# microsoft/VidTok

Measured on NVIDIA H100. Metric: frames/sec encode+decode, kl_causal_488 17x256x256, higher is better.
Workload: dtype bf16

## Files before the change

### vidtok_b200/csrc/conv_tc.cu

```cuda
#include <cuda.h>

#include <cstdio>
#include <cstdlib>
#include <cstring>
#include <mutex>
#include <string>
#include <type_traits>

#include "common.cuh"
#include "kernels.h"
#include "tc_host.h"
#include "tc_ptx.cuh"

namespace vt {

namespace {

thread_local std::string g_tc_err;

struct TcParams {
  int B, To, Ho, Wo, Co, Ti;
  int BW, BH, BT;
  int tilesW, tilesH, tilesT;
  int num_n_tiles, BN;
  long long num_tiles;
  int kt, kh, kw, Ci, num_kc;
  int st, pt, ph, pw, to_off;
  int sp;
  int t_mode, cacheT;
  int stages;
  const float* bias;
  int res_mode;
  const bf16* res;
  long long rsB, rsT, rsH, rsW;
  int resT, res_t_mode, res_pool_off;
  const bf16* res_cache;
  float ra, rb;
  void* out;
  long long osB, osT, osH, osW, osC;
  int out_f32;
  int Co_real;
  int w_batched;
  int ln_mode, ln_silu;
  const float* ln_gamma;
  const float* ln_beta;
  void* out2;
  int res_mma;
  int halo, hP, a_stages;
  uint32_t halo_bytes;
  int split, a_lo, b_lo, o_lo;
  float acc_scale;
  int kparts;
  int reg_mode, reg_zc, reg_sample;
  const float* reg_noise;
  float* reg_z;
  int* reg_idx;
  double* reg_kl;
  FsqConst reg_fsq;
  uint32_t misc_off;
  int stage_out;
  uint32_t stage_smem;
  uint32_t stage_off;
  int half_dim, half_ext;
  int relu;
};

struct TcMaps {
  CUtensorMap a[4];
  CUtensorMap c;
  CUtensorMap b;
  CUtensorMap r;
  CUtensorMap e;
  CUtensorMap o, o2;
};

constexpr int kConsumerWarps = 8;
constexpr int kProducerWarp = kConsumerWarps;
constexpr int kThreads = (kConsumerWarps + 4) * 32;
constexpr int kABytes = 128 * 128;
constexpr uint32_t kBarTurn = 3, kBarBias = 5, kBarStage = 7;
constexpr uint32_t kStageOutBytes = 64 * 128;

__host__ __device__ constexpr bool ping_pong(int BN, bool split) { return !split && (BN == 64 || BN == 128); }

using namespace tcx;

struct TileCoord {
  int b, t0, h0, w0, n0;
};
__device__ __forceinline__ TileCoord decode_tile(const TcParams& p, long long tile) {
  TileCoord c;
  const int nt = (int)(tile % p.num_n_tiles);
  long long m = tile / p.num_n_tiles;
  const int tw = (int)(m % p.tilesW); m /= p.tilesW;
  const int th = (int)(m % p.tilesH); m /= p.tilesH;
  const int tt = (int)(m % p.tilesT);
  c.b = (int)(m / p.tilesT);
  c.t0 = tt * p.BT; c.h0 = th * p.BH; c.w0 = tw * p.BW; c.n0 = nt * p.BN;
  return c;
}
__device__ __forceinline__ bool tap_time(const TcParams& p, const TileCoord& tc, int a, int& tv, bool& from_cache) {
  tv = (tc.t0 + p.to_off) * p.st + a - p.pt;
  from_cache = false;
  if (tv + p.BT <= 0) {
    if (p.t_mode == 0) return false;
    if (p.t_mode == 1) { tv = 0; return true; }
    from_cache = true;
    tv = p.cacheT + tv;
    return true;
  }
  return true;
}
__device__ __forceinline__ int tile_taps(const TcParams& p, const TileCoord& tc) {
  int n = 0;
  for (int a = 0; a < p.kt; ++a) {
    int tv;
    bool from_cache;
    if (tap_time(p, tc, a, tv, from_cache)) ++n;
  }
  return n;
}

__device__ __forceinline__ float quad_sum(float v) {
  v += __shfl_xor_sync(0xffffffffu, v, 1);
  v += __shfl_xor_sync(0xffffffffu, v, 2);
  return v;
}

template <int BN, bool kSplit, bool kStage = false>
__global__ void __launch_bounds__(kThreads, 1)
conv_tc_kernel(const __grid_constant__ TcMaps maps, const TcParams p) {
  extern __shared__ uint8_t smem_raw[];
  const uint32_t smem_base = (smem_u32(smem_raw) + 1023u) & ~1023u;
  uint8_t* smem_gen = smem_raw + (smem_base - smem_u32(smem_raw));
  const int warp = threadIdx.x >> 5, lane = threadIdx.x & 31;
  const uint32_t a_bytes = kABytes;
  constexpr uint32_t b_bytes = (uint32_t)BN * 128u;
  constexpr uint32_t kPl = kSplit ? 2u : 1u;
  const uint32_t stage_bytes = kPl * (p.halo ? b_bytes : a_bytes + b_bytes);
  const uint32_t win_bytes = kPl * p.halo_bytes;
  const uint32_t ring_base = smem_base + (p.halo ? (uint32_t)p.a_stages * win_bytes : 0u);
  const uint32_t bar_base = ring_base + p.stages * stage_bytes + p.stage_smem;
  auto full_bar = [&](int s) { return bar_base + 8u * s; };
  auto empty_bar = [&](int s) { return bar_base + 8u * (p.stages + s); };
  auto fullA_bar = [&](int s) { return bar_base + 8u * (2 * p.stages + s); };
  auto emptyA_bar = [&](int s) { return bar_base + 8u * (2 * p.stages + p.a_stages + s); };
  constexpr bool kPingPong = ping_pong(BN, kSplit);
  float* sbias = reinterpret_cast<float*>(smem_gen + p.misc_off);
  float* rowbuf = sbias + 2 * 768;

  if (threadIdx.x == 0) {
    constexpr uint32_t readers = kPingPong ? kConsumerWarps / 2 : kConsumerWarps;
    for (int s = 0; s < p.stages; ++s) {
      mbar_init(full_bar(s), 1);
      mbar_init(empty_bar(s), readers);
    }
    for (int s = 0; s < p.a_stages; ++s) {
      mbar_init(fullA_bar(s), 1);
      mbar_init(emptyA_bar(s), readers);
    }
    asm volatile("fence.mbarrier_init.release.cluster;" ::: "memory");
  }
  __syncthreads();

  const int nsp = p.kh * p.kw;
  const int num_kc = p.num_kc, nstages = p.stages;
  const bool halo = p.halo != 0;
  const int res_steps = p.res_mma ? BN / 64 : 0;

  if (warp >= kProducerWarp) {
    asm volatile("setmaxnreg.dec.sync.aligned.u32 40;" ::: "memory");
    if (warp != kProducerWarp) return;
    const bool el = elect_one();
    if (el) {
      prefetch_tmap(&maps.a[0]);
      prefetch_tmap(&maps.b);
      if (p.sp == 2) { prefetch_tmap(&maps.a[1]); prefetch_tmap(&maps.a[2]); prefetch_tmap(&maps.a[3]); }
      if (p.t_mode == 2) prefetch_tmap(&maps.c);
      if (p.res_mma) { prefetch_tmap(&maps.r); prefetch_tmap(&maps.e); }
    }
    int stage = 0, sA = 0;
    uint32_t phase = 0, phA = 0;
    auto acquire = [&](uint32_t bytes) {
      mbar_wait(empty_bar(stage), phase ^ 1u);
      if (el) mbar_expect_tx(full_bar(stage), bytes);
    };
    auto advance = [&]() { if (++stage == nstages) { stage = 0; phase ^= 1u; } };
    auto load_b_planes = [&](uint32_t dst, const CUtensorMap* m, int kcol, int n, int wb_) {
      tma_load_3d(dst, m, full_bar(stage), kcol, n, wb_);
      if constexpr (kSplit) tma_load_3d(dst + b_bytes, m, full_bar(stage), p.b_lo + kcol, n, wb_);
    };
    auto load_window = [&](const CUtensorMap* m, int c0, int lo_off, int cw, int ch, int ct, int cb) {
      mbar_wait(emptyA_bar(sA), phA ^ 1u);
      if (el) {
        mbar_expect_tx(fullA_bar(sA), win_bytes);
        tma_load_5d(smem_base + (uint32_t)sA * win_bytes, m, fullA_bar(sA), c0, cw, ch, ct, cb);
        if constexpr (kSplit) tma_load_5d(smem_base + (uint32_t)sA * win_bytes + p.halo_bytes, m, fullA_bar(sA), lo_off + c0, cw, ch, ct, cb);
      }
      if (++sA == p.a_stages) { sA = 0; phA ^= 1u; }
    };
    for (long long tile = blockIdx.x; tile < p.num_tiles; tile += gridDim.x) {
      const TileCoord tc = decode_tile(p, tile);
      const int wb = p.w_batched ? tc.b : 0;
      for (int a = 0; a < p.kt; ++a) {
        int tv;
        bool from_cache;
        if (!tap_time(p, tc, a, tv, from_cache)) continue;
        if (halo) {
          const CUtensorMap* mapA = from_cache ? &maps.c : &maps.a[0];
          for (int kc = 0; kc < num_kc; ++kc) {
            load_window(mapA, kc * 64, p.a_lo, tc.w0 - p.pw, tc.h0 - p.ph, tv, tc.b);
            int kcol = a * nsp * p.Ci + kc * 64;
            for (int sp = 0; sp < nsp; ++sp, kcol += p.Ci) {
              acquire(stage_bytes);
              if (el) load_b_planes(ring_base + stage * stage_bytes, &maps.b, kcol, tc.n0, wb);
              advance();
            }
          }
        } else {
          int kcol = a * nsp * p.Ci;
          for (int bb = 0; bb < p.kh; ++bb) {
            for (int c = 0; c < p.kw; ++c, kcol += p.Ci) {
              const int dh = bb - p.ph, dw2 = c - p.pw;
              int ch, cw;
              const CUtensorMap* mapA;
              if (p.sp == 2) {
                mapA = &maps.a[(dh & 1) * 2 + (dw2 & 1)];
                ch = tc.h0 + (dh >> 1);
                cw = tc.w0 + (dw2 >> 1);
              } else {
                mapA = &maps.a[0];
                ch = tc.h0 + dh;
                cw = tc.w0 + dw2;
              }
              if (from_cache) mapA = &maps.c;
              for (int kc = 0; kc < num_kc; ++kc) {
                acquire(stage_bytes);
                if (el) {
                  const uint32_t sa = smem_base + stage * stage_bytes;
                  tma_load_5d(sa, mapA, full_bar(stage), kc * 64, cw, ch, tv, tc.b);
                  if constexpr (kSplit) tma_load_5d(sa + a_bytes, mapA, full_bar(stage), p.a_lo + kc * 64, cw, ch, tv, tc.b);
                  load_b_planes(sa + kPl * a_bytes, &maps.b, kcol + kc * 64, tc.n0, wb);
                }
                advance();
              }
            }
          }
        }
      }
      for (int g = 0; g < res_steps; ++g) {
        if (halo) {
          load_window(&maps.r, tc.n0 + g * 64, p.o_lo, tc.w0 - p.pw, tc.h0 - p.ph, tc.t0, tc.b);
          acquire(b_bytes);
          if (el) tma_load_3d(ring_base + stage * stage_bytes, &maps.e, full_bar(stage), g * 64, 0, 0);
        } else {
          acquire(kPl * a_bytes + b_bytes);
          if (el) {
            const uint32_t sa = smem_base + stage * stage_bytes;
            tma_load_5d(sa, &maps.r, full_bar(stage), tc.n0 + g * 64, tc.w0, tc.h0, tc.t0, tc.b);
            if constexpr (kSplit) tma_load_5d(sa + a_bytes, &maps.r, full_bar(stage), p.o_lo + tc.n0 + g * 64, tc.w0, tc.h0, tc.t0, tc.b);
            tma_load_3d(sa + kPl * a_bytes, &maps.e, full_bar(stage), g * 64, 0, 0);
          }
        }
        advance();
      }
    }
    return;
  }

  asm volatile("setmaxnreg.inc.sync.aligned.u32 232;" ::: "memory");
  constexpr int R = BN / 2;
  constexpr int kHalves = kPingPong ? 2 : 1;
  constexpr bool kSum = kSplit && BN <= 128;
  const int g = warp >> 2, wq = warp & 3;
  const bool leader = lane == 0;
  const uint32_t hi_b = desc_hi(1024u);
  const uint32_t hi_a = halo ? desc_hi((uint32_t)p.hP * 128u) : hi_b;
  const uint32_t a_half = halo ? 8u * (uint32_t)p.hP * 128u : 64u * 128u;
  const uint32_t a_row_off = kPingPong ? 0u : (uint32_t)g * a_half;
  const uint32_t a_pl = halo ? p.halo_bytes : a_bytes;
  const uint32_t b_addr0 = halo ? ring_base : smem_base + kPl * a_bytes;
  float acc[kHalves][R];
  float sum[kSum ? R : 1];
  int stage = 0, sA = 0, sR = 0;
  uint32_t phase = 0, phA = 0;
  int pend_stage = -1;
  bool pend_win = false;
  auto release = [&]() {
    if (leader) {
      if (pend_stage >= 0) mbar_arrive(empty_bar(pend_stage));
      if (pend_win) mbar_arrive(emptyA_bar(sR));
    }
    if (pend_win && ++sR == p.a_stages) sR = 0;
    pend_stage = -1;
    pend_win = false;
  };
  auto kstep = [&](bool a_from_stage, uint32_t a_addr, uint32_t scale, bool res, bool last_of_window) {
    mbar_wait(full_bar(stage), phase);
    if (a_from_stage) a_addr = smem_base + stage * stage_bytes + a_row_off;
    const uint32_t b_addr = b_addr0 + stage * stage_bytes;
    const uint32_t al = desc_lo(a_addr), bl = desc_lo(b_addr);
    wgmma_fence();
#pragma unroll
    for (uint32_t j = 0; j < 4u; ++j) {
      const uint64_t ah = desc(al + 2u * j, hi_a), bh = desc(bl + 2u * j, hi_b);
      wgmma_k16<BN, kSplit>(acc[0], ah, bh, j == 0 ? scale : 1u);
      if constexpr (kPingPong) wgmma_k16<BN, kSplit>(acc[1], desc(al + (a_half >> 4) + 2u * j, hi_a), bh, j == 0 ? scale : 1u);
      if constexpr (kSplit) {
        wgmma_k16<BN, kSplit>(acc[0], desc(al + (a_pl >> 4) + 2u * j, hi_a), bh, 1u);
        if (!res) wgmma_k16<BN, kSplit>(acc[0], ah, desc(bl + (b_bytes >> 4) + 2u * j, hi_b), 1u);
      }
    }
    wgmma_commit();
    wgmma_wait<1>();
    release();
    pend_stage = stage;
    pend_win = last_of_window;
    if (++stage == nstages) { stage = 0; phase ^= 1u; }
  };

  const int rbase = (kPingPong ? 0 : 64 * g) + 16 * wq + (lane >> 2);
  const int cq = 2 * (lane & 3);
  const bool res_direct = (p.res_mode == 1 && !p.res_mma);
  const bool store_a = (p.ln_mode != 1);
  const float inv_n = 1.0f / (float)BN;
  int last_n0 = -1;
  uint32_t cbuf = 1;

  int owner = 0;
  for (long long tile = blockIdx.x; tile < p.num_tiles; tile += gridDim.x, owner ^= 1) {
    const TileCoord tc = decode_tile(p, tile);
    if constexpr (kPingPong) {
      if (owner != g) {
        const int taps = tile_taps(p, tc);
        stage += taps * nsp * num_kc + res_steps;
        if ((stage / nstages) & 1) phase ^= 1u;
        stage %= nstages;
        if (halo) {
          const int nw = taps * num_kc + res_steps;
          sA += nw;
          if ((sA / p.a_stages) & 1) phA ^= 1u;
          sA %= p.a_stages;
          sR = (sR + nw) % p.a_stages;
        }
        continue;
      }
      if (tile != blockIdx.x) named_bar_sync(kBarTurn + g, kConsumerWarps * 32);
    }
    uint32_t G = 0xFFFFFFFFu;
    if constexpr (kSum) {
      if (p.kparts > 1) {
        const uint32_t nk = (uint32_t)(tile_taps(p, tc) * nsp * num_kc + res_steps);
        G = (nk + (uint32_t)p.kparts - 1u) / (uint32_t)p.kparts;
      }
#pragma unroll
      for (int i = 0; i < R; ++i) sum[i] = 0.f;
    }
    uint32_t ks = 0, accum = 0;
    auto step = [&](bool a_from_stage, uint32_t a_addr, bool res, bool last_of_window) {
      if constexpr (kSum) {
        if (ks > 0 && ks % G == 0) {
          wgmma_wait<0>();
          acc_fence(acc[0]);
          release();
#pragma unroll
          for (int i = 0; i < R; ++i) sum[i] += acc[0][i];
          accum = 0;
        }
      }
      kstep(a_from_stage, a_addr, accum, res, last_of_window);
      accum = 1;
      ++ks;
    };
    for (int a = 0; a < p.kt; ++a) {
      int tv;
      bool from_cache;
      if (!tap_time(p, tc, a, tv, from_cache)) continue;
      if (halo) {
        for (int kc = 0; kc < num_kc; ++kc) {
          mbar_wait(fullA_bar(sA), phA);
          const uint32_t win = smem_base + (uint32_t)sA * win_bytes + a_row_off;
          for (int bb = 0; bb < p.kh; ++bb)
            for (int c = 0; c < p.kw; ++c)
              step(false, win + (uint32_t)(bb * p.hP + c) * 128u, false, bb == p.kh - 1 && c == p.kw - 1);
          if (++sA == p.a_stages) { sA = 0; phA ^= 1u; }
        }
      } else {
        for (int s = nsp * num_kc; s > 0; --s) step(true, 0u, false, false);
      }
    }
    for (int gr = 0; gr < res_steps; ++gr) {
      if (halo) {
        mbar_wait(fullA_bar(sA), phA);
        step(false, smem_base + (uint32_t)sA * win_bytes + a_row_off + (uint32_t)(p.ph * p.hP + p.pw) * 128u, true, true);
        if (++sA == p.a_stages) { sA = 0; phA ^= 1u; }
      } else {
        step(true, 0u, true, false);
      }
    }
    if constexpr (kPingPong) {
      if (tile + gridDim.x < p.num_tiles) named_bar_arrive(kBarTurn + (g ^ 1), kConsumerWarps * 32);
    }
    wgmma_wait<0>();
#pragma unroll
    for (int hf = 0; hf < kHalves; ++hf) acc_fence(acc[hf]);
    release();
    if constexpr (kSum) {
#pragma unroll
      for (int i = 0; i < R; ++i) acc[0][i] += sum[i];
    }

    if (tc.n0 != last_n0) {
      last_n0 = tc.n0;
      cbuf ^= 1u;
      constexpr int nthr = kPingPong ? 128 : kConsumerWarps * 32;
      float* b_ = sbias + ((kPingPong ? 2 * g : 0) + cbuf) * 768;
      for (int i = threadIdx.x % nthr; i < BN; i += nthr) {
        b_[i] = (p.bias && tc.n0 + i < p.Co_real) ? p.bias[tc.n0 + i] : 0.f;
        if (p.ln_mode) { const float sc = (p.ln_silu && !kSplit) ? 0.5f : 1.0f; b_[256 + i] = sc * p.ln_gamma[tc.n0 + i]; b_[512 + i] = sc * p.ln_beta[tc.n0 + i]; }
      }
      named_bar_sync(kPingPong ? kBarBias + g : 1u, nthr);
    }
    const float* bias_s = sbias + ((kPingPong ? 2 * g : 0) + cbuf) * 768;
    const float* gamma_s = bias_s + 256;
    const float* beta_s = bias_s + 512;

#pragma unroll
    for (int hf = 0; hf < kHalves; ++hf) {
      float (&acc_h)[R] = acc[hf];
      int row0 = rbase + 64 * hf;
      asm volatile("" : "+r"(row0));
      bool valid[2];
      long long ooff[2];
      auto row_geom = [&](int row, int& t, int& h, int& w) {
        const int dw = halo ? (row & 7) : row % p.BW;
        const int dh = halo ? (row >> 3) : (row / p.BW) % p.BH;
        const int dt = halo ? 0 : row / (p.BW * p.BH);
        t = tc.t0 + dt; h = tc.h0 + dh; w = tc.w0 + dw;
        return (t < p.To) && (h < p.Ho) && (w < p.Wo);
      };
#pragma unroll
      for (int r = 0; r < 2; ++r) {
        int t, h, w;
        valid[r] = row_geom(row0 + 8 * r, t, h, w);
        ooff[r] = (long long)tc.b * p.osB + (long long)t * p.osT + (long long)h * p.osH + (long long)w * p.osW;
      }
      auto res_pair = [&](const bf16* rp, int c, float& x0, float& x1) {
        const uint32_t hw = *reinterpret_cast<const uint32_t*>(rp + c);
        if constexpr (kSplit) {
          const uint32_t lw = *reinterpret_cast<const uint32_t*>(rp + p.o_lo + c);
          x0 = f16_lo(hw) + f16_lo(lw);
          x1 = f16_hi(hw) + f16_hi(lw);
        } else {
          x0 = bf16_lo(hw);
          x1 = bf16_hi(hw);
        }
      };
#pragma unroll
      for (int j = 0; j < BN / 8; ++j) {
        const int c = 8 * j + cq;
#pragma unroll
        for (int e = 0; e < 4; ++e) {
          float f = kSplit ? fmaf(acc_h[4 * j + e], p.acc_scale, bias_s[c + (e & 1)]) : acc_h[4 * j + e] + bias_s[c + (e & 1)];
          if (p.rb != 1.0f) f *= p.rb;
          acc_h[4 * j + e] = f;
        }
      }
      if (res_direct || p.res_mode == 3) {
#pragma unroll
        for (int r = 0; r < 2; ++r) {
          int t, h, w;
          if (!row_geom(row0 + 8 * r, t, h, w)) continue;
          const bf16* r0 = nullptr;
          const bf16* r1 = nullptr;
          const bf16* r2 = nullptr;
          if (res_direct) {
            r0 = p.res + (long long)tc.b * p.rsB + (long long)t * p.rsT + (long long)h * p.rsH + (long long)w * p.rsW + tc.n0;
          } else {
            const long long sp = (long long)tc.b * p.rsB + (long long)h * p.rsH + (long long)w * p.rsW + tc.n0;
            const int ta = 2 * t - 1 + p.res_pool_off, tb = ta + 1, tcn = ta + 2;
            if (ta >= 0) r0 = p.res + sp + (long long)ta * p.rsT;
            else if (p.res_t_mode == 1) r0 = p.res + sp;
            else if (p.res_t_mode == 2) r0 = p.res_cache + (((long long)tc.b * p.Ho + h) * p.Wo + w) * (long long)p.Co * (kSplit ? 2 : 1) + tc.n0;
            if (tb < p.resT) r1 = p.res + sp + (long long)tb * p.rsT;
            if (tcn < p.resT) r2 = p.res + sp + (long long)tcn * p.rsT;
          }
#pragma unroll
          for (int j = 0; j < BN / 8; ++j) {
            const int c = 8 * j + cq;
            if (res_direct) {
              float x0, x1;
              res_pair(r0, c, x0, x1);
              acc_h[4 * j + 2 * r] = fmaf(p.ra, x0, acc_h[4 * j + 2 * r]);
              acc_h[4 * j + 2 * r + 1] = fmaf(p.ra, x1, acc_h[4 * j + 2 * r + 1]);
            } else {
              float s0 = 0.f, s1 = 0.f, x0, x1;
              if (r0) { res_pair(r0, c, x0, x1); s0 += x0; s1 += x1; }
              if (r1) { res_pair(r1, c, x0, x1); s0 += x0; s1 += x1; }
              if (r2) { res_pair(r2, c, x0, x1); s0 += x0; s1 += x1; }
              const float s3 = p.ra * (1.0f / 3.0f);
              acc_h[4 * j + 2 * r] = fmaf(s3, s0, acc_h[4 * j + 2 * r]);
              acc_h[4 * j + 2 * r + 1] = fmaf(s3, s1, acc_h[4 * j + 2 * r + 1]);
            }
          }
        }
      }
      if (p.relu) {
#pragma unroll
        for (int i = 0; i < R; ++i) acc_h[i] = acc_h[i] < 0.f ? 0.f : acc_h[i];
      }

      if (p.out_f32) {
        if (p.out) {
#pragma unroll
          for (int r = 0; r < 2; ++r) {
            if (!valid[r]) continue;
            float* of = reinterpret_cast<float*>(p.out) + ooff[r];
#pragma unroll
            for (int j = 0; j < BN / 8; ++j)
#pragma unroll
              for (int e = 0; e < 2; ++e) {
                const int n = tc.n0 + 8 * j + cq + e;
                if (n < p.Co_real) of[(long long)n * p.osC] = acc_h[4 * j + 2 * r + e];
              }
          }
        }
        if (p.reg_mode) {
          if constexpr (BN == 32) {
#pragma unroll
            for (int j = 0; j < 4; ++j)
#pragma unroll
              for (int e = 0; e < 4; ++e) rowbuf[(rbase + 8 * (e >> 1)) * 33 + 8 * j + cq + (e & 1)] = acc_h[4 * j + e];
            asm volatile("bar.sync 2, %0;" ::"n"(kConsumerWarps * 32) : "memory");
            if (threadIdx.x < 128) {
              const int row = threadIdx.x;
              float f[32];
#pragma unroll
              for (int c = 0; c < 32; ++c) f[c] = rowbuf[row * 33 + c];
              int t, h, w;
              const bool ok = row_geom(row, t, h, w);
              const long long plane = p.osC;
              const long long pos = (long long)t * p.osT + (long long)h * p.osH + (long long)w * p.osW;
              if (p.reg_mode == 1) {
                float part = 0.f;
                auto kl_row = [&](auto ZC) {
                  constexpr int zc = decltype(ZC)::value;
                  const long long zb = (long long)tc.b * zc * plane + pos;
#pragma unroll
                  for (int c = 0; c < zc; ++c) {
                    float zv;
                    part += kl_sample_one(f[c], f[zc + c], p.reg_sample ? p.reg_noise[zb + c * plane] : 0.f, p.reg_sample, zv);
                    p.reg_z[zb + c * plane] = zv;
                  }
                };
                if (ok) {
                  if (p.reg_zc == 4) kl_row(std::integral_constant<int, 4>());
                  else if (p.reg_zc == 8) kl_row(std::integral_constant<int, 8>());
                  else kl_row(std::integral_constant<int, 16>());
                }
                double dsum = (double)part;
#pragma unroll
                for (int o = 16; o > 0; o >>= 1) dsum += __shfl_xor_sync(0xffffffffu, dsum, o);
                if (lane == 0) atomicAdd(p.reg_kl, dsum);
              } else if (ok) {
                const long long zb = (long long)tc.b * p.reg_zc * plane + pos;
                float idx = 0.f;
#pragma unroll
                for (int c = 0; c < VT_MAX_FSQ; ++c)
                  if (c < p.reg_zc) p.reg_z[zb + c * plane] = fsq_code(p.reg_fsq, c, f[c], idx);
                if (p.reg_idx) p.reg_idx[(long long)tc.b * plane + pos] = (int)idx;
              }
            }
            asm volatile("bar.sync 2, %0;" ::"n"(kConsumerWarps * 32) : "memory");
          }
        }
        continue;
      }

      if constexpr (kStage) {
        static_assert(!kSplit && BN == 256, "staged stores: the cooperative bf16 schedule");
        {
          float rstd[2], nmr[2];
#pragma unroll
          for (int r = 0; r < 2; ++r) {
            float s = 0.f, q = 0.f;
#pragma unroll
            for (int j = 0; j < BN / 8; ++j) {
              const float f0 = acc_h[4 * j + 2 * r], f1 = acc_h[4 * j + 2 * r + 1];
              s += f0 + f1;
              q = fmaf(f0, f0, q);
              q = fmaf(f1, f1, q);
              const uint32_t kp = pack_bf16x2(f0, f1);
              acc_h[4 * j + 2 * r] = bf16_lo(kp);
              acc_h[4 * j + 2 * r + 1] = bf16_hi(kp);
            }
            const float mean = quad_sum(s) * inv_n;
            float var = fmaf(-mean, mean, quad_sum(q) * inv_n);
            var = var < 0.f ? 0.f : var;
            rstd[r] = rsqrtf(var + 1e-6f);
            nmr[r] = -mean * rstd[r];
          }
          const uint32_t sbuf = smem_base + p.stage_off + (uint32_t)(row0 >> 6) * kStageOutBytes;
          const uint32_t sw = sbuf + swz128_unit(row0 & 63, 0) + 2u * cq;
          auto put_s = [&](int r, int u, uint32_t word) {
            asm volatile("st.shared.b32 [%0], %1;" ::"r"((sw ^ ((uint32_t)u << 4)) + 1024u * r), "r"(word) : "memory");
          };
          const bool issuer = (threadIdx.x & 127) == 0;
          auto reserve = [&]() {
            if (issuer) bulk_wait_read<0>();
            named_bar_sync(kBarStage + g, 128);
          };
          auto send = [&](const CUtensorMap* m, int k) {
            fence_async_smem();
            named_bar_sync(kBarStage + g, 128);
            if (issuer) {
              const int ho = g * p.half_ext;
              tma_store_5d(m, sbuf, tc.n0 + 64 * k, tc.w0 + (p.half_dim == 1 ? ho : 0), tc.h0 + (p.half_dim == 2 ? ho : 0),
                           tc.t0 + (p.half_dim == 3 ? ho : 0), tc.b);
              bulk_commit();
            }
          };
          if (store_a) {
#pragma unroll
            for (int k = 0; k < BN / 64; ++k) {
              reserve();
#pragma unroll
              for (int r = 0; r < 2; ++r)
#pragma unroll
                for (int u = 0; u < 8; ++u) put_s(r, u, pack_bf16x2(acc_h[4 * (8 * k + u) + 2 * r], acc_h[4 * (8 * k + u) + 2 * r + 1]));
              send(&maps.o, k);
            }
          }
          if (p.ln_mode) {
            const CUtensorMap* nmap = p.ln_mode == 1 ? &maps.o : &maps.o2;
#pragma unroll
            for (int k = 0; k < BN / 64; ++k) {
              reserve();
#pragma unroll
              for (int r = 0; r < 2; ++r)
#pragma unroll
                for (int u = 0; u < 8; ++u) {
                  const int j = 8 * k + u, c = 8 * j + cq;
                  float y0 = fmaf(fmaf(acc_h[4 * j + 2 * r], rstd[r], nmr[r]), gamma_s[c], beta_s[c]);
                  float y1 = fmaf(fmaf(acc_h[4 * j + 2 * r + 1], rstd[r], nmr[r]), gamma_s[c + 1], beta_s[c + 1]);
                  if (p.ln_silu) {
                    y0 = fmaf(y0, tanh_approx(y0), y0);
                    y1 = fmaf(y1, tanh_approx(y1), y1);
                  }
                  put_s(r, u, pack_bf16x2(y0, y1));
                }
              send(nmap, k);
            }
          }
          continue;
        }
      }

      auto put = [&](void* optr, int r, int c, float y0, float y1) {
        bf16* o = reinterpret_cast<bf16*>(optr) + ooff[r] + tc.n0 + c;
        if constexpr (kSplit) {
          const uint32_t hw = pack_f16x2(y0, y1);
          *reinterpret_cast<uint32_t*>(o) = hw;
          *reinterpret_cast<uint32_t*>(o + p.o_lo) = pack_f16x2(y0 - f16_lo(hw), y1 - f16_hi(hw));
        } else {
          *reinterpret_cast<uint32_t*>(o) = pack_bf16x2(y0, y1);
        }
      };
      if constexpr (kSplit) {
        if (store_a) {
#pragma unroll
          for (int r = 0; r < 2; ++r)
            if (valid[r])
#pragma unroll
              for (int j = 0; j < BN / 8; ++j) put(p.out, r, 8 * j + cq, acc_h[4 * j + 2 * r], acc_h[4 * j + 2 * r + 1]);
        }
        if (p.ln_mode) {
          void* nout = p.ln_mode == 1 ? p.out : p.out2;
#pragma unroll
          for (int r = 0; r < 2; ++r) {
            float s = 0.f;
#pragma unroll
            for (int j = 0; j < BN / 8; ++j) s += acc_h[4 * j + 2 * r] + acc_h[4 * j + 2 * r + 1];
            const float mean = quad_sum(s) * inv_n;
            float q = 0.f;
#pragma unroll
            for (int j = 0; j < BN / 8; ++j) {
              const float d0 = acc_h[4 * j + 2 * r] - mean, d1 = acc_h[4 * j + 2 * r + 1] - mean;
              q = fmaf(d0, d0, q);
              q = fmaf(d1, d1, q);
            }
            const float rstd = 1.0f / sqrtf(quad_sum(q) * inv_n + 1e-6f);
            if (!valid[r]) continue;
#pragma unroll
            for (int j = 0; j < BN / 8; ++j) {
              const int c = 8 * j + cq;
              float y0 = (acc_h[4 * j + 2 * r] - mean) * rstd * gamma_s[c] + beta_s[c];
              float y1 = (acc_h[4 * j + 2 * r + 1] - mean) * rstd * gamma_s[c + 1] + beta_s[c + 1];
              if (p.ln_silu) { y0 = silu_tc(y0); y1 = silu_tc(y1); }
              put(nout, r, c, y0, y1);
            }
          }
        }
      } else {
#pragma unroll
        for (int r = 0; r < 2; ++r) {
          float s = 0.f, q = 0.f;
#pragma unroll
          for (int j = 0; j < BN / 8; ++j) {
            const float f0 = acc_h[4 * j + 2 * r], f1 = acc_h[4 * j + 2 * r + 1];
            s += f0 + f1;
            q = fmaf(f0, f0, q);
            q = fmaf(f1, f1, q);
            const uint32_t kp = pack_bf16x2(f0, f1);
            if (store_a && valid[r]) *reinterpret_cast<uint32_t*>(reinterpret_cast<bf16*>(p.out) + ooff[r] + tc.n0 + 8 * j + cq) = kp;
            acc_h[4 * j + 2 * r] = bf16_lo(kp);
            acc_h[4 * j + 2 * r + 1] = bf16_hi(kp);
          }
          if (!p.ln_mode) continue;
          const float mean = quad_sum(s) * inv_n;
          float var = fmaf(-mean, mean, quad_sum(q) * inv_n);
          var = var < 0.f ? 0.f : var;
          const float rstd = rsqrtf(var + 1e-6f);
          const float nmr = -mean * rstd;
          if (!valid[r]) continue;
          void* nout = p.ln_mode == 1 ? p.out : p.out2;
#pragma unroll
          for (int j = 0; j < BN / 8; ++j) {
            const int c = 8 * j + cq;
            float y0 = fmaf(fmaf(acc_h[4 * j + 2 * r], rstd, nmr), gamma_s[c], beta_s[c]);
            float y1 = fmaf(fmaf(acc_h[4 * j + 2 * r + 1], rstd, nmr), gamma_s[c + 1], beta_s[c + 1]);
            if (p.ln_silu) {
              y0 = fmaf(y0, tanh_approx(y0), y0);
              y1 = fmaf(y1, tanh_approx(y1), y1);
            }
            put(nout, r, c, y0, y1);
          }
        }
      }
    }
  }
  if (kStage && (threadIdx.x & 127) == 0) bulk_wait<0>();
}

__global__ void fill_identity_kernel(bf16* e, int f16, float value) {
  const int r = blockIdx.x, c = threadIdx.x;
  if (f16) reinterpret_cast<__half*>(e)[r * 256 + c] = __float2half_rn(r == c ? value : 0.0f);
  else e[r * 256 + c] = __float2bfloat16_rn(r == c ? value : 0.0f);
}

bool choose_tile(const ConvP& p, int rows, int& BW, int& BH, int& BT) {
  const bool allow_bt = (p.st == 1) && (p.t_mode == 0);
  long long best = -1;
  auto ceil_to = [](int v, int b) { return (long long)((v + b - 1) / b) * b; };
  for (int bw = 128; bw >= 8; bw >>= 1) {
    for (int bh = rows / bw; bh >= 1; bh >>= 1) {
      if (bh > 256) continue;
      const int bt = rows / (bw * bh);
      if (bt > 1 && !allow_bt) continue;
      if (bt > 16) continue;
      const long long padded = ceil_to(p.Wo, bw) * ceil_to(p.Ho, bh) * ceil_to(p.To, bt);
      const long long cost = padded * 1024 + (long long)(bw > 16 ? bw - 16 : 16 - bw) * 4 + (bt - 1);
      if (best < 0 || cost < best) { best = cost; BW = bw; BH = bh; BT = bt; }
    }
  }
  return best >= 0;
}
int choose_bn(int Co) {
  for (int bn = 256; bn >= 32; bn >>= 1)
    if (Co % bn == 0) return bn;
  return 0;
}

cudaError_t identity_tiles(int dev, bool split, cudaStream_t s, const bf16** out) {
  static bf16* ident_dev[2][kMaxDevices] = {{nullptr}};
  static std::mutex ident_mu;
  const int ik = split ? 1 : 0;
  std::lock_guard<std::mutex> lock(ident_mu);
  if (!ident_dev[ik][dev]) {
    cudaStreamCaptureStatus cap = cudaStreamCaptureStatusNone;
    if (cudaStreamIsCapturing(s, &cap) != cudaSuccess || cap != cudaStreamCaptureStatusNone) {
      cudaGetLastError();
      g_tc_err = "the residual identity tiles do not exist yet and the stream is capturing";
      return cudaErrorStreamCaptureUnsupported;
    }
    const int nmat = split ? 16 : 1;
    bf16* e = nullptr;
    cudaError_t err = cudaMalloc(&e, (size_t)nmat * 256 * 256 * sizeof(bf16));
    if (err != cudaSuccess) { g_tc_err = "cudaMalloc(identity)"; return err; }
    for (int i = 0; i < nmat; ++i) fill_identity_kernel<<<256, 256, 0, s>>>(e + (size_t)i * 256 * 256, ik, ldexpf(1.0f, i));
    if ((err = cudaStreamSynchronize(s)) != cudaSuccess) { cudaFree(e); g_tc_err = "identity fill"; return err; }
    ident_dev[ik][dev] = e;
  }
  *out = ident_dev[ik][dev];
  return cudaSuccess;
}

}

const char* conv_tc_last_error() { return g_tc_err.c_str(); }

cudaError_t conv_tc_prepare_identity(cudaStream_t s) {
  int dev = 0;
  if (cudaError_t e = current_device(dev)) return e;
  const bf16* unused;
  for (int split = 0; split < 2; ++split)
    if (cudaError_t e = identity_tiles(dev, split != 0, s, &unused)) return e;
  return cudaSuccess;
}

bool conv_tc_plan(const ConvP& p, DType tout, const TcLnFusion* ln, const TcRegFusion* reg, int w_batches, TcPlan* out) {
  g_tc_err.clear();
  auto no = [&](const char* why) { g_tc_err = why; return false; };
  if (p.Ci % 64 != 0) return no("Cin % 64 != 0");
  const int Co_pad = (p.Co + 31) / 32 * 32;
  if (choose_bn(Co_pad) == 0) return no("Cout has no valid N tile");
  const bool split = p.split != 0;
  const long long cw = split ? 2 : 1;
  if (split ? (tout == DT_BF16) : (tout == DT_SPLIT)) return no("activation layout of input and output differ");
  if (p.isC != 1 || p.isW != cw * p.Ci || p.isH != (long long)p.Wi * cw * p.Ci || p.isT != (long long)p.Hi * p.Wi * cw * p.Ci) return no("input is not dense channels-last");
  if (p.isB % 8 != 0) return no("batch stride not 16-byte aligned");
  if (tout != DT_F32) {
    if (p.Co % 32 != 0) return no("bf16 output needs Cout % 32 == 0");
    if (p.osC != 1 || p.osW % 8 != 0 || p.osH % 8 != 0 || p.osT % 8 != 0 || p.osB % 8 != 0) return no("output rows are not 16-byte aligned channels-last");
  }
  if (!((p.sh == 1 && p.sw == 1) || (p.sh == 2 && p.sw == 2))) return no("spatial stride");
  if (p.sh == 2 && ((p.Hi | p.Wi) & 1)) return no("stride-2 needs even H, W");
  if (p.st != 1 && p.st != 2) return no("time stride");
  if (p.ut != 1 || p.uh != 1 || p.uw != 1 || p.t_rep != 0) return no("folded upsampling / replicate prefix");
  if (p.res_mode != 0 && p.res_mode != 1 && p.res_mode != 3) return no("residual mode");
  if (p.res_mode != 0 && tout == DT_F32) return no("residual with fp32 output");
  if (p.t_mode == 2 && p.sh != 1) return no("cache mode with spatial stride");
  if (p.Wi > 65535 || p.Hi > 65535) return no("extent");
  if (w_batches > 1 && w_batches != p.B) return no("batched weights need one weight matrix per batch element");
  if (p.relu && ((ln && ln->mode) || (reg && reg->mode))) return no("ReLU with a fused LayerNorm or regularizer epilogue");
  TcPlan t = TcPlan();
  t.p = p; t.tout = tout; t.w_batches = w_batches;
  const int nk = p.kt * p.kh * p.kw * (p.Ci / 64);
  if (ln && ln->mode) {
    if (tout != DT_F32 && p.Co <= 256 && choose_bn(p.Co) == p.Co && (!split || p.Co <= 128 || nk < 16)) t.ln = *ln;
    else g_tc_err = "fused LayerNorm needs one N tile covering Cout, a 16-bit output and (split) Cout <= 128 or < 16 K steps";
  }
  if (reg && reg->mode) {
    const int need = reg->mode == 1 ? 2 * reg->zc : reg->zc;
    const bool zc_ok = reg->mode == 1 ? (reg->zc == 4 || reg->zc == 8 || reg->zc == 16) : reg->zc <= VT_MAX_FSQ;
    if (tout == DT_F32 && Co_pad == 32 && need <= p.Co && zc_ok && p.osW == 1) t.reg = *reg;
    else g_tc_err = "regularizer epilogue needs an fp32 [B,C,T,H,W] head with Cout <= 32 holding all latent channels";
  }
  auto plan = [&](bool allow_halo, int bn_cap) -> int {
    t.halo = 0; t.hP = 0; t.a_stages = 0; t.halo_bytes = 0;
    t.BN = choose_bn(Co_pad);
    if (bn_cap && t.BN > bn_cap) t.BN = bn_cap;
    if (!choose_tile(p, 128, t.BW, t.BH, t.BT)) { g_tc_err = "no tile shape"; return -1; }
    const bool geom = p.sh == 1 && p.sw == 1 && p.kh * p.kw > 1 && p.kh <= 3 && p.kw <= 3 && p.Ho == p.Hi && p.Wo == p.Wi &&
                      w_batches <= 1 && p.Wo % 8 == 0 && p.Ho % 16 == 0;
    if (allow_halo && geom) {
      t.halo = 1;
      t.BW = 8; t.BH = 16; t.BT = 1;
      t.hP = 16;
      t.halo_bytes = (uint32_t)((16 + p.kh - 1) * t.hP * 128);
      t.a_stages = 2;
    }
    const size_t stage_bytes = (size_t)cw * ((t.halo ? 0 : (size_t)kABytes) + (size_t)t.BN * 128);
    const size_t budget = 225 * 1024;
    const size_t a_ring = (size_t)t.a_stages * t.halo_bytes * cw;
    const size_t misc = (ping_pong(t.BN, split) ? 4 : 2) * 768 * 4 + (t.reg.mode ? 128 * 33 * 4 : 0);
    const size_t fixed = 1024  + misc + 16;
    if (budget < fixed + a_ring + 2 * (stage_bytes + 16)) return 1;
    int stages = (int)((budget - fixed - a_ring) / (stage_bytes + 16));
    if (stages > 8) stages = 8;
    static const int cap = [] { const char* e = getenv("VT_TC_STAGES"); return e ? atoi(e) : 0; }();
    if (cap >= 2 && stages > cap) stages = cap;
    t.stages = stages;
    const size_t bars = 8 * (2 * (size_t)stages + 2 * (size_t)t.a_stages);
    const size_t staging = 2 * (size_t)kStageOutBytes;
    const bool staged = !split && tout == DT_BF16 && t.BN == 256 &&
                        1024 + ((a_ring + stages * stage_bytes + staging + bars + 15) & ~(size_t)15) + misc <= 227 * 1024;
    t.stage_out = staged ? 1 : 0;
    t.misc_off = (uint32_t)((a_ring + stages * stage_bytes + (staged ? staging : 0) + bars + 15) & ~(size_t)15);
    t.smem = 1024 + t.misc_off + misc;
    t.kparts = (split && t.BN <= 128 && nk >= 16) ? (nk >= 64 ? 8 : 4) : 1;
    return 0;
  };
  const bool need_row = t.ln.mode != 0;
  const int bn_pref = (split && !need_row && w_batches <= 1) ? (nk >= 128 ? 64 : (nk >= 16 ? 128 : 0)) : 0;
  int rc = plan(true, bn_pref);
  if (rc == 1) rc = plan(false, bn_pref);
  if (rc == 1 && !need_row) rc = plan(false, 128);
  if (rc == 1) return no("not enough shared memory for 2 stages");
  if (rc != 0) return false;
  bool ident_ok = true;
  if (split) {
    const float ws = p.acc_scale != 0.f ? 1.0f / p.acc_scale : 1.0f;
    t.ident_s = ilogbf(ws);
    ident_ok = t.ident_s >= 0 && t.ident_s <= 15 && ldexpf(1.0f, t.ident_s) == ws;
  }
  t.res_mma = (ident_ok && p.res_mode == 1 && p.ra == 1.0f && p.rb == 1.0f && t.BN % 64 == 0 && p.Co % 64 == 0 && p.rsW % 8 == 0 &&
               p.rsH % 8 == 0 && p.rsT % 8 == 0 && p.rsB % 8 == 0 && (((uintptr_t)p.res) & 15) == 0) ? 1 : 0;
  *out = t;
  return true;
}

cudaError_t launch_conv_tc(const TcPlan& pl, const bf16* x, const bf16* w_nk, void* out, cudaStream_t s, long long w_batch_stride) {
  if (!tmap_encoder()) { g_tc_err = "cuTensorMapEncodeTiled unavailable"; return cudaErrorNotSupported; }
  const ConvP& p = pl.p;
  const TcRegFusion& reg = pl.reg;
  const bool split = p.split != 0;
  const int cw = split ? 2 : 1;
  if (reg.mode ? (!reg.z || (reg.mode == 1 && (!reg.kl_acc || (reg.sample && !reg.noise)))) : !out) { g_tc_err = "null output"; return cudaErrorInvalidValue; }
  if (p.t_mode == 2 && (!p.cache || p.cacheT <= 0)) { g_tc_err = "cache mode without cache"; return cudaErrorInvalidValue; }
  int dev = 0;
  const cudaError_t dev_err = current_device(dev);
  if (dev_err != cudaSuccess) { g_tc_err = "no current device, or its index is out of range"; return dev_err; }
  const int Co_pad = (p.Co + 31) / 32 * 32, Kpad = p.kt * p.kh * p.kw * p.Ci;
  TcParams t;
  memset(&t, 0, sizeof(t));
  t.BW = pl.BW; t.BH = pl.BH; t.BT = pl.BT; t.BN = pl.BN;
  t.halo = pl.halo; t.hP = pl.hP; t.a_stages = pl.a_stages; t.halo_bytes = pl.halo_bytes;
  t.stages = pl.stages; t.misc_off = pl.misc_off; t.kparts = pl.kparts; t.res_mma = pl.res_mma;
  t.stage_smem = pl.stage_out ? 2 * kStageOutBytes : 0;
  t.stage_off = (uint32_t)pl.a_stages * pl.halo_bytes + (uint32_t)pl.stages * (uint32_t)((pl.halo ? 0 : kABytes) + pl.BN * 128);
  t.stage_out = (pl.stage_out && ((uintptr_t)out & 15) == 0 && ((uintptr_t)pl.ln.out2 & 15) == 0) ? 1 : 0;
  t.tilesW = (p.Wo + t.BW - 1) / t.BW; t.tilesH = (p.Ho + t.BH - 1) / t.BH; t.tilesT = (p.To + t.BT - 1) / t.BT;
  t.num_n_tiles = Co_pad / t.BN;
  t.num_tiles = (long long)p.B * t.tilesT * t.tilesH * t.tilesW * t.num_n_tiles;
  t.split = split ? 1 : 0; t.a_lo = p.Ci; t.b_lo = Kpad; t.o_lo = pl.o_lo ? pl.o_lo : p.Co;
  t.acc_scale = (split && p.acc_scale != 0.f) ? p.acc_scale : 1.0f;
  t.B = p.B; t.To = p.To; t.Ho = p.Ho; t.Wo = p.Wo; t.Co = p.Co; t.Ti = p.Ti;
  t.kt = p.kt; t.kh = p.kh; t.kw = p.kw; t.Ci = p.Ci; t.num_kc = p.Ci / 64;
  t.st = p.st; t.pt = p.pt; t.ph = p.ph; t.pw = p.pw; t.to_off = p.to_off; t.sp = p.sh;
  t.t_mode = p.t_mode; t.cacheT = p.cacheT;
  t.bias = p.bias; t.res_mode = p.res_mode; t.res = (const bf16*)p.res;
  t.rsB = p.rsB; t.rsT = p.rsT; t.rsH = p.rsH; t.rsW = p.rsW; t.resT = p.resT; t.res_t_mode = p.res_t_mode; t.res_pool_off = p.res_pool_off;
  t.res_cache = (const bf16*)p.res_cache; t.ra = p.ra; t.rb = p.rb;
  t.out = out; t.osB = p.osB; t.osT = p.osT; t.osH = p.osH; t.osW = p.osW; t.osC = p.osC;
  t.out_f32 = (pl.tout == DT_F32) ? 1 : 0;
  t.Co_real = p.Co;
  t.ln_mode = pl.ln.mode; t.ln_silu = pl.ln.silu ? 1 : 0; t.ln_gamma = pl.ln.gamma; t.ln_beta = pl.ln.beta; t.out2 = pl.ln.out2;
  if (reg.mode) {
    t.reg_mode = reg.mode; t.reg_zc = reg.zc; t.reg_sample = reg.sample; t.reg_noise = reg.noise; t.reg_z = reg.z;
    t.reg_idx = reg.indices; t.reg_kl = reg.kl_acc;
    if (reg.mode == 2) t.reg_fsq = make_fsq_const(reg.zc, reg.fsq_levels);
  }
  t.w_batched = pl.w_batches > 1 ? 1 : 0;
  t.relu = p.relu ? 1 : 0;

  TcMaps maps;
  auto encode_act = [&](CUtensorMap* m, const bf16* base, int Wn, int Hn, long long sw_, long long sh_, int Tn, long long st_, long long bs) -> bool {
    cuuint64_t dims[5] = {(cuuint64_t)(cw * p.Ci), (cuuint64_t)Wn, (cuuint64_t)Hn, (cuuint64_t)Tn, (cuuint64_t)p.B};
    cuuint64_t strides[4] = {(cuuint64_t)sw_ * 2, (cuuint64_t)sh_ * 2, (cuuint64_t)st_ * 2, (cuuint64_t)bs * 2};
    cuuint32_t box[5] = {64, (cuuint32_t)t.BW, (cuuint32_t)t.BH, (cuuint32_t)t.BT, 1};
    if (t.halo) { box[1] = (cuuint32_t)t.hP; box[2] = (cuuint32_t)(16 + p.kh - 1); }
    return encode_tmap_16b(m, 5, base, dims, strides, box, "activation", g_tc_err);
  };
  if (p.sh == 1) {
    if (!encode_act(&maps.a[0], x, p.Wi, p.Hi, p.isW, p.isH, p.Ti, p.isT, p.isB)) return cudaErrorInvalidValue;
    maps.a[1] = maps.a[2] = maps.a[3] = maps.a[0];
  } else {
    for (int hp = 0; hp < 2; ++hp)
      for (int wp = 0; wp < 2; ++wp)
        if (!encode_act(&maps.a[hp * 2 + wp], x + (long long)hp * p.isH + (long long)wp * p.isW, (p.Wi - wp + 1) / 2,
                        (p.Hi - hp + 1) / 2, 2 * p.isW, 2 * p.isH, p.Ti, p.isT, p.isB))
          return cudaErrorInvalidValue;
  }
  if (p.t_mode == 2) {
    if (!encode_act(&maps.c, (const bf16*)p.cache, p.Wi, p.Hi, p.isW, p.isH, p.cacheT, p.isT, (long long)p.cacheT * p.Hi * p.Wi * p.Ci * cw)) return cudaErrorInvalidValue;
  } else {
    maps.c = maps.a[0];
  }
  {
    const int nb = pl.w_batches > 1 ? pl.w_batches : 1;
    cuuint64_t dims[3] = {(cuuint64_t)(cw * Kpad), (cuuint64_t)Co_pad, (cuuint64_t)nb};
    cuuint64_t strides[2] = {(cuuint64_t)(cw * Kpad) * 2, (cuuint64_t)(nb > 1 ? w_batch_stride : (long long)cw * Kpad * Co_pad) * 2};
    cuuint32_t box[3] = {64, (cuuint32_t)t.BN, 1};
    if (!encode_tmap_16b(&maps.b, 3, w_nk, dims, strides, box, "weights", g_tc_err)) return cudaErrorInvalidValue;
  }
  auto encode_out = [&](CUtensorMap* m, const void* base, int Tn, long long sW, long long sH, long long sT, long long sB, int bw, int bh, int bt) -> bool {
    cuuint64_t dims[5] = {(cuuint64_t)(cw * p.Co), (cuuint64_t)p.Wo, (cuuint64_t)p.Ho, (cuuint64_t)Tn, (cuuint64_t)p.B};
    cuuint64_t strides[4] = {(cuuint64_t)sW * 2, (cuuint64_t)sH * 2, (cuuint64_t)sT * 2, (cuuint64_t)sB * 2};
    cuuint32_t box[5] = {64, (cuuint32_t)bw, (cuuint32_t)bh, (cuuint32_t)bt, 1};
    return encode_tmap_16b(m, 5, base, dims, strides, box, "output/residual", g_tc_err);
  };
  maps.r = maps.a[0]; maps.e = maps.b;
  if (t.res_mma) {
    const bf16* ident = nullptr;
    if (cudaError_t err = identity_tiles(dev, split, s, &ident)) return err;
    ident += (size_t)pl.ident_s * 256 * 256;
    if (!encode_out(&maps.r, p.res, p.resT, p.rsW, p.rsH, p.rsT, p.rsB, t.halo ? t.hP : t.BW, t.halo ? 16 + p.kh - 1 : t.BH, t.BT)) return cudaErrorInvalidValue;
    cuuint64_t dims[3] = {256, 256, 1};
    cuuint64_t strides[2] = {512, 256 * 512};
    cuuint32_t box[3] = {64, (cuuint32_t)t.BN, 1};
    if (!encode_tmap_16b(&maps.e, 3, ident, dims, strides, box, "identity", g_tc_err)) return cudaErrorInvalidValue;
  }
  if (t.stage_out) {
    int hb[3] = {t.BW, t.BH, t.BT};
    t.half_dim = t.BT > 1 ? 3 : (t.BH > 1 ? 2 : 1);
    t.half_ext = (hb[t.half_dim - 1] /= 2);
    if (!encode_out(&maps.o, out, p.To, p.osW, p.osH, p.osT, p.osB, hb[0], hb[1], hb[2])) return cudaErrorInvalidValue;
    maps.o2 = maps.o;
    if (t.ln_mode == 2 && !encode_out(&maps.o2, t.out2, p.To, p.osW, p.osH, p.osT, p.osB, hb[0], hb[1], hb[2])) return cudaErrorInvalidValue;
  } else {
    maps.o = maps.o2 = maps.a[0];
  }
  {
    static SmemLimitOnce smem_limit;
    cudaError_t e = smem_limit.ensure(dev, 227 * 1024, conv_tc_kernel<32, false>, conv_tc_kernel<64, false>, conv_tc_kernel<128, false>,
                                      conv_tc_kernel<256, false>, conv_tc_kernel<32, true>, conv_tc_kernel<64, true>,
                                      conv_tc_kernel<128, true>, conv_tc_kernel<256, true>, conv_tc_kernel<256, false, true>);
    if (e != cudaSuccess) { g_tc_err = "cudaFuncSetAttribute(smem)"; return e; }
  }
  const int num_sms = device_sms(dev);
  const unsigned grid = (unsigned)(t.num_tiles < num_sms ? t.num_tiles : num_sms);
  const double Mrows = (double)p.B * p.To * p.Ho * p.Wo;
  char det[192] = "";
  if (prof_enabled()) {
    char pad[48] = "";
    const int pt_back = time_pad_back(p);
    int n = 0;
    if (p.pt != (p.kt - 1) + (1 - p.st) || pt_back != 0) n = snprintf(pad, sizeof(pad), " pad%d.%d", p.pt, pt_back);
    if (p.res_mode == 3 && p.res_pool_off != 0) snprintf(pad + n, sizeof(pad) - n, " pool%d", p.res_pool_off);
    snprintf(det, sizeof(det), "k%d%d%d s%d%d %d->%d @%dx%dx%d tile%dx%dx%d bn%d%s ln%d r%d%s p%d t%d st%d%s%s", p.kt, p.kh, p.kw, p.st, p.sh, p.Ci, p.Co, p.To, p.Ho, p.Wo, t.BT, t.BH, t.BW, t.BN, t.halo ? " halo" : "", t.ln_mode, p.res_mode, t.res_mma ? "m" : "", split ? t.kparts : 1, p.t_mode, t.stages, pad, p.relu ? " relu" : "");
  }
  ProfScope _ps(split ? "conv_tc3" : "conv_tc", 2.0 * Mrows * p.kt * p.kh * p.kw * p.Ci * p.Co,
                2.0 * cw * ((double)p.B * p.Ti * p.Hi * p.Wi * p.Ci) + Mrows * p.Co * (pl.tout == DT_F32 ? 4.0 : 2.0 * cw), s, det);
  auto launch = [&](auto kern) { kern<<<grid, kThreads, pl.smem, s>>>(maps, t); };
  if (t.stage_out) launch(conv_tc_kernel<256, false, true>);
  else switch (t.BN * 2 + (split ? 1 : 0)) {
    case 64: launch(conv_tc_kernel<32, false>); break;
    case 65: launch(conv_tc_kernel<32, true>); break;
    case 128: launch(conv_tc_kernel<64, false>); break;
    case 129: launch(conv_tc_kernel<64, true>); break;
    case 256: launch(conv_tc_kernel<128, false>); break;
    case 257: launch(conv_tc_kernel<128, true>); break;
    case 512: launch(conv_tc_kernel<256, false>); break;
    default: launch(conv_tc_kernel<256, true>); break;
  }
  count_launch();
  return cudaGetLastError();
}

}
```

Baseline: 472.0.

## Load residual tiles unpadded and pack two residual steps per halo window slot

In the halo path, the residual input used to be loaded as a full padded halo window, one window slot per residual step. It is now loaded as an exact BW x BH x BT tile, and two consecutive residual k-steps share one A-window stage. The goal is to cut residual TMA bytes and window-ring turnover. The consumer's descriptor layout, offsets, stage-skip accounting and the tensor-map box all change to match, so the producer/consumer phase bookkeeping has to stay consistent for odd res_steps and for ping-pong.

```diff
diff --git a/vidtok_b200/csrc/conv_tc.cu b/vidtok_b200/csrc/conv_tc.cu
--- a/vidtok_b200/csrc/conv_tc.cu
+++ b/vidtok_b200/csrc/conv_tc.cu
@@ -250,7 +250,16 @@
       }
       for (int g = 0; g < res_steps; ++g) {
         if (halo) {
-          load_window(&maps.r, tc.n0 + g * 64, p.o_lo, tc.w0 - p.pw, tc.h0 - p.ph, tc.t0, tc.b);
+          if ((g & 1) == 0) {
+            mbar_wait(emptyA_bar(sA), phA ^ 1u);
+            if (el) mbar_expect_tx(fullA_bar(sA), (g + 1 < res_steps ? 2u : 1u) * kPl * a_bytes);
+          }
+          if (el) {
+            const uint32_t dst = smem_base + (uint32_t)sA * win_bytes + (uint32_t)(g & 1) * a_bytes;
+            tma_load_5d(dst, &maps.r, fullA_bar(sA), tc.n0 + g * 64, tc.w0, tc.h0, tc.t0, tc.b);
+            if constexpr (kSplit) tma_load_5d(dst + p.halo_bytes, &maps.r, fullA_bar(sA), p.o_lo + tc.n0 + g * 64, tc.w0, tc.h0, tc.t0, tc.b);
+          }
+          if (((g & 1) || g + 1 == res_steps) && ++sA == p.a_stages) { sA = 0; phA ^= 1u; }
           acquire(b_bytes);
           if (el) tma_load_3d(ring_base + stage * stage_bytes, &maps.e, full_bar(stage), g * 64, 0, 0);
         } else {
@@ -296,6 +305,8 @@
     pend_win = false;
   };
   auto kstep = [&](bool a_from_stage, uint32_t a_addr, uint32_t scale, bool res, bool last_of_window) {
+    const uint32_t ha = res ? hi_b : hi_a;
+    const uint32_t half = res ? 64u * 128u : a_half;
     mbar_wait(full_bar(stage), phase);
     if (a_from_stage) a_addr = smem_base + stage * stage_bytes + a_row_off;
     const uint32_t b_addr = b_addr0 + stage * stage_bytes;
@@ -303,11 +314,11 @@
     wgmma_fence();
 #pragma unroll
     for (uint32_t j = 0; j < 4u; ++j) {
-      const uint64_t ah = desc(al + 2u * j, hi_a), bh = desc(bl + 2u * j, hi_b);
+      const uint64_t ah = desc(al + 2u * j, ha), bh = desc(bl + 2u * j, hi_b);
       wgmma_k16<BN, kSplit>(acc[0], ah, bh, j == 0 ? scale : 1u);
-      if constexpr (kPingPong) wgmma_k16<BN, kSplit>(acc[1], desc(al + (a_half >> 4) + 2u * j, hi_a), bh, j == 0 ? scale : 1u);
+      if constexpr (kPingPong) wgmma_k16<BN, kSplit>(acc[1], desc(al + (half >> 4) + 2u * j, ha), bh, j == 0 ? scale : 1u);
       if constexpr (kSplit) {
-        wgmma_k16<BN, kSplit>(acc[0], desc(al + (a_pl >> 4) + 2u * j, hi_a), bh, 1u);
+        wgmma_k16<BN, kSplit>(acc[0], desc(al + (a_pl >> 4) + 2u * j, ha), bh, 1u);
         if (!res) wgmma_k16<BN, kSplit>(acc[0], ah, desc(bl + (b_bytes >> 4) + 2u * j, hi_b), 1u);
       }
     }
@@ -319,8 +330,8 @@
     if (++stage == nstages) { stage = 0; phase ^= 1u; }
   };
 
+  const int cq = 2 * (lane & 3);
   const int rbase = (kPingPong ? 0 : 64 * g) + 16 * wq + (lane >> 2);
-  const int cq = 2 * (lane & 3);
   const bool res_direct = (p.res_mode == 1 && !p.res_mma);
   const bool store_a = (p.ln_mode != 1);
   const float inv_n = 1.0f / (float)BN;
@@ -337,7 +348,7 @@
         if ((stage / nstages) & 1) phase ^= 1u;
         stage %= nstages;
         if (halo) {
-          const int nw = taps * num_kc + res_steps;
+          const int nw = taps * num_kc + (res_steps + 1) / 2;
           sA += nw;
           if ((sA / p.a_stages) & 1) phA ^= 1u;
           sA %= p.a_stages;
@@ -391,9 +402,10 @@
     }
     for (int gr = 0; gr < res_steps; ++gr) {
       if (halo) {
-        mbar_wait(fullA_bar(sA), phA);
-        step(false, smem_base + (uint32_t)sA * win_bytes + a_row_off + (uint32_t)(p.ph * p.hP + p.pw) * 128u, true, true);
-        if (++sA == p.a_stages) { sA = 0; phA ^= 1u; }
+        if ((gr & 1) == 0) mbar_wait(fullA_bar(sA), phA);
+        const bool last = (gr & 1) || gr + 1 == res_steps;
+        step(false, smem_base + (uint32_t)sA * win_bytes + (uint32_t)(gr & 1) * a_bytes + (kPingPong ? 0u : (uint32_t)g * 64u * 128u), true, last);
+        if (last && ++sA == p.a_stages) { sA = 0; phA ^= 1u; }
       } else {
         step(true, 0u, true, false);
       }
@@ -985,7 +997,7 @@
     const bf16* ident = nullptr;
     if (cudaError_t err = identity_tiles(dev, split, s, &ident)) return err;
     ident += (size_t)pl.ident_s * 256 * 256;
-    if (!encode_out(&maps.r, p.res, p.resT, p.rsW, p.rsH, p.rsT, p.rsB, t.halo ? t.hP : t.BW, t.halo ? 16 + p.kh - 1 : t.BH, t.BT)) return cudaErrorInvalidValue;
+    if (!encode_out(&maps.r, p.res, p.resT, p.rsW, p.rsH, p.rsT, p.rsB, t.BW, t.BH, t.BT)) return cudaErrorInvalidValue;
     cuuint64_t dims[3] = {256, 256, 1};
     cuuint64_t strides[2] = {512, 256 * 512};
     cuuint32_t box[3] = {64, (cuuint32_t)t.BN, 1};
```

Result: no change. 474.7 (median of 6 runs) (+0.6%).
